# zyc-123/InstanceDiff

Measured on AMD Instinct MI355X. Metric: denoising steps/sec (256x256 bs16), higher is better.
Workload: dtype f32; 1 GPU; 256x256 1-ch synthetic, 1000-step reverse chain, batch 16 per GPU, 2 UNet fwd + reverse update per step; global_batch=16, parallelism=replicas x1 (no collective)

## Files before the change

instancediff_amd/csrc/conv_wino4.hip:

```cpp
#include "conv_args.h"
#include "wino_common.h"

using idiff_detail::ConvArgs;

namespace {

using namespace idiff_wino;

constexpr int CK = 4;
constexpr int TW = 32, TH = 16;
constexpr int RCOLS = TW + 2;
constexpr int RS = 40;
constexpr int TRH = TH + 2;
constexpr int PS = TRH * RS;
constexpr int PSP = 768;
constexpr int NT = 512;
constexpr int NL = 6;
constexpr int R_FLOATS = NL * NT;
constexpr int V_FLOATS = 9 * 2 * 64 * 4;
constexpr int U_FLOATS = 9 * 4 * 64 * 4;

typedef float floatx2 __attribute__((ext_vector_type(2)));

template <bool UPSAMPLED>
constexpr unsigned long long chunk_live() {
    unsigned long long m = 0;
    for (int q = 0; q < 9; ++q) m |= (unsigned long long)quad_live<UPSAMPLED>(q) << (4 * q);
    return m;
}
template <bool UPSAMPLED>
constexpr unsigned chunk_sets() {
    unsigned m = 0, n = 0;
    for (int q = 0; q < 9; ++q) m |= (n & 1u) << q, n += quad_live<UPSAMPLED>(q) != 0;
    return m | (n & 1u) << 9;
}

struct Geo4 {
    int np;
    int total;
    int tiles_y8;
};

#ifdef IDIFF_WINO_SLOTS
#define SLOT_INIT long long sl_acc[10] = {0, 0, 0, 0, 0, 0, 0, 0, 0, 0}, sl_t = 0;
#define SLOT_START sl_t = __builtin_readcyclecounter();
#define SLOT_MARK(k)                                        \
    {                                                       \
        const long long t_ = __builtin_readcyclecounter();  \
        sl_acc[k] += t_ - sl_t;                             \
        sl_t = t_;                                          \
    }
#define SLOT_FINI                                                                                                                   \
    if (lane == 0) {                                                                                                                \
        long long w_ = 0;                                                                                                           \
        for (int q_ = 0; q_ < 9; ++q_) w_ += sl_acc[q_];                                                                            \
        atomicAdd((unsigned long long*)trace + 8 + 2 * wave, (unsigned long long)w_);                                               \
        atomicAdd((unsigned long long*)trace + 9 + 2 * wave, (unsigned long long)sl_acc[9]);                                        \
    }
#else
#define SLOT_INIT
#define SLOT_START
#define SLOT_MARK(k)
#define SLOT_FINI
#endif

template <int MODE, int SPEC, bool RAG, bool HEAVY, bool G16>
__device__ __forceinline__ void conv_wino4_body(const ConvArgs& a, const Geo4& g, float* smem TRACE_PARAM) {
    static_assert(!G16 || (MODE == IDIFF_CONV_NORMAL && SPEC != 2), "the 16-byte gather: contiguous pieces, LDS-DMA only");
    constexpr int HU = G16 ? 5 : 4, HR = 3;
    constexpr int N_U = HEAVY ? HU : 9 - HU;
    constexpr int NR = G16 ? (HEAVY ? HR : 3 - HR) : NL;
    constexpr bool UPS = MODE == IDIFF_CONV_UPSAMPLE2;
    float* const Rb = smem;
    float* const Vb = smem + 3 * R_FLOATS;
    float* const Ub = Vb + 2 * V_FLOATS;
    float* const econst = Ub + 2 * U_FLOATS;
    int* const gtab = reinterpret_cast<int*>(econst + 512);
    constexpr unsigned R_BYTES = R_FLOATS * 4, U_BYTES = U_FLOATS * 4;
    const unsigned lds_base = __builtin_amdgcn_readfirstlane((unsigned)reinterpret_cast<unsigned long long>(smem));
    const unsigned U_LDS0 = lds_base + (3 * R_FLOATS + 2 * V_FLOATS) * 4;

    const int tid = threadIdx.x;
    const int lane = tid & 63;
    const int wave = __builtin_amdgcn_readfirstlane(tid >> 6);
    const int k4 = lane >> 4;
    const int cb = wave & 3;
    const int tblk = wave >> 2;
    const int g16_u0 = HEAVY ? wave : 4 * HU + wave - 4, g16_r0 = HEAVY ? wave : 4 * HR + wave - 4;
    const int HWin = a.Hin * a.Win;
    const int nchunks = a.Cin / CK;

    constexpr int RSRC_FLAGS = 0x00020000;
    struct View {
        int b, co0, y0, x0;
    };
    const float *p0A = a.src0, *p1A = a.src0, *puA = a.wwino4, *p0B = a.src0, *p1B = a.src0, *puB = a.wwino4;
    View vA = {0, 0, 0, 0}, vB = {0, 0, 0, 0};
    int nrB = 0;
    unsigned omaskA = 0, omaskB = 0;
    int it_b = 0, it_cob = 0, it_px = 0, it_py = 0;
    const int tiles_y = g.np / a.tiles_x;
    int d_cob, d_px, d_py, d_b;
    {
        const int G0 = gridDim.x;
        d_cob = G0 % a.ncob;
        const int r1 = G0 / a.ncob;
        d_px = r1 % a.tiles_x;
        const int r2 = r1 / a.tiles_x;
        d_py = r2 % tiles_y;
        d_b = r2 / tiles_y;
    }
    auto decode_first = [&](int item) {
        it_cob = item % a.ncob;
        const int r1 = item / a.ncob;
        it_px = r1 % a.tiles_x;
        const int r2 = r1 / a.tiles_x;
        it_py = r2 % tiles_y;
        it_b = r2 / tiles_y;
    };
    auto advance_item = [&]() {
        it_cob += d_cob;
        int carry = it_cob >= a.ncob;
        it_cob -= carry ? a.ncob : 0;
        it_px += d_px + carry;
        carry = it_px >= a.tiles_x;
        it_px -= carry ? a.tiles_x : 0;
        it_py += d_py + carry;
        carry = it_py >= tiles_y;
        it_py -= carry ? tiles_y : 0;
        it_b += d_b + carry;
    };
    auto decode_B = [&]() {
        vB.b = it_b, vB.co0 = it_cob * 64, vB.y0 = it_py * TH, vB.x0 = it_px * TW;
        puB = scalar_ptr(a.wwino4 + (long long)it_cob * U_FLOATS);
        p0B = scalar_ptr(a.src0 + (long long)it_b * a.bs0);
        p1B = scalar_ptr(SPEC == 3 ? a.src1 + (long long)it_b * a.bs1 : a.src0);
        nrB = 0x7fffffff;
    };
    auto write_table = [&](const View& v) {
        unsigned om;
        if (G16) gather_decode16<NT, NR, 256, PSP / 4, PS / 4, RS / 4>(tid, g16_r0 * 64 + lane, om, v.y0, v.x0, a, gtab, HWin);
        else gather_decode<MODE, NT, NL, PSP, PS, RS, RCOLS>(tid, om, v.y0, v.x0, a, gtab, HWin);
        return om;
    };
    auto shift_B_to_A = [&]() { p0A = p0B, p1A = p1B, puA = puB, vA = vB, omaskA = omaskB; };
    const int ustride_b = a.ncob * U_FLOATS * 4;

    typedef const __attribute__((address_space(4))) floatx4* cfloatx4p;
    struct Pro {
        floatx4 a, b;
    };
    auto load_pro = [&](int p) {
        Pro r;
        if (SPEC == 2) {
            const bool inA = p < nchunks;
            const long long o = (long long)(inA ? vA.b : vB.b) * a.C0r + (inA ? p : p - nchunks) * CK;
            r.a = *(cfloatx4p)(a.pro_a + o);
            r.b = *(cfloatx4p)(a.pro_b + o);
        }
        return r;
    };

    const unsigned u_voff = tid * 16;
    const unsigned l_voff = lane * 16;
    auto dma_u_piece16 = [&](int p, int buf, int i) {
        const bool inA = p < nchunks;
        const unsigned ub = (unsigned)(g16_u0 + 4 * i) * 1024u;
        const int so = (inA ? p : p - nchunks) * ustride_b + (int)ub;
        const __amdgpu_buffer_rsrc_t rsu = __builtin_amdgcn_make_buffer_rsrc(const_cast<float*>(inA ? puA : puB), 0, inA ? 0x7fffffff : nrB, RSRC_FLAGS);
        const unsigned lds0 = __builtin_amdgcn_readfirstlane(U_LDS0 + (unsigned)buf * U_BYTES + ub);
        asm volatile("s_nop 4\n\ts_mov_b32 m0, %2\n\ts_nop 0\n\tbuffer_load_dwordx4 %0, %1, %3 offen lds" ::"v"(l_voff), "s"(rsu), "s"(lds0), "s"(so) : "memory");
    };
    auto dma_u = [&](int p, int buf) {
        if (G16) {
#pragma unroll
            for (int i = 0; i < N_U; ++i) dma_u_piece16(p, buf, i);
            return;
        }
        const bool inA = p < nchunks;
        const int so = (inA ? p : p - nchunks) * ustride_b;
        const __amdgpu_buffer_rsrc_t rsu = __builtin_amdgcn_make_buffer_rsrc(const_cast<float*>(inA ? puA : puB), 0, inA ? 0x7fffffff : nrB, RSRC_FLAGS);
        const unsigned lds0 = __builtin_amdgcn_readfirstlane(U_LDS0 + (unsigned)buf * U_BYTES + (unsigned)wave * 1024u);
        asm volatile(
            "s_nop 4\n\ts_mov_b32 m0, %2\n\ts_nop 0\n\tbuffer_load_dwordx4 %0, %1, %3 offen lds\n\t"
            "s_add_u32 m0, m0, 0x2000\n\ts_nop 0\n\tbuffer_load_dwordx4 %0, %1, %4 offen lds\n\t"
            "s_add_u32 m0, m0, 0x2000\n\ts_nop 0\n\tbuffer_load_dwordx4 %0, %1, %5 offen lds\n\t"
            "s_add_u32 m0, m0, 0x2000\n\ts_nop 0\n\tbuffer_load_dwordx4 %0, %1, %6 offen lds"
            ::"v"(u_voff), "s"(rsu), "s"(lds0), "s"(so), "s"(so + NT * 16), "s"(so + 2 * NT * 16), "s"(so + 3 * NT * 16)
            : "memory", "scc");
        if (!HEAVY) {
            const unsigned lds4 = __builtin_amdgcn_readfirstlane(lds0 + 4 * NT * 16 - 256 * 16);
            asm volatile("s_nop 4\n\ts_mov_b32 m0, %2\n\ts_nop 0\n\tbuffer_load_dwordx4 %0, %1, %3 offen lds" ::"v"(u_voff), "s"(rsu), "s"(lds4),
                         "s"(so + 4 * NT * 16 - 256 * 16)
                         : "memory");
        }
    };
    auto dma_u_piece = [&](int p, int buf, int i) {
        if (G16) return dma_u_piece16(p, buf, i);
        const bool inA = p < nchunks;
        const int so = (inA ? p : p - nchunks) * ustride_b + (i < 4 ? i * NT * 16 : 4 * NT * 16 - 256 * 16);
        const __amdgpu_buffer_rsrc_t rsu = __builtin_amdgcn_make_buffer_rsrc(const_cast<float*>(inA ? puA : puB), 0, inA ? 0x7fffffff : nrB, RSRC_FLAGS);
        const unsigned lds0 = __builtin_amdgcn_readfirstlane(U_LDS0 + (unsigned)buf * U_BYTES + (unsigned)wave * 1024u + (unsigned)(i < 4 ? i * NT * 16 : 4 * NT * 16 - 256 * 16));
        asm volatile("s_nop 4\n\ts_mov_b32 m0, %2\n\ts_nop 0\n\tbuffer_load_dwordx4 %0, %1, %3 offen lds" ::"v"(u_voff), "s"(rsu), "s"(lds0), "s"(so) : "memory");
    };
    auto dma_raw = [&](int p, unsigned rslot) {
        const bool inA = p < nchunks;
        const int cbase = (inA ? p : p - nchunks) * CK;
        int goff[NL];
#pragma unroll
        for (int i = 0; i < NL; ++i) goff[i] = gtab[i * NT + tid];
        const int C0v = a.C0v;
        const bool second = SPEC == 3 && cbase >= C0v;
        const unsigned long long b0 = reinterpret_cast<unsigned long long>(inA ? p0A : p0B), b1 = reinterpret_cast<unsigned long long>(inA ? p1A : p1B);
        const float* const base = reinterpret_cast<const float*>(second ? b1 : b0);
        const int so = (second ? cbase - C0v : cbase) * HWin * 4;
        const __amdgpu_buffer_rsrc_t rs = __builtin_amdgcn_make_buffer_rsrc(const_cast<float*>(base), 0, inA ? 0x7fffffff : nrB, RSRC_FLAGS);
        const unsigned lds0 = __builtin_amdgcn_readfirstlane(lds_base + rslot + (unsigned)wave * 256u);
        asm volatile(
            "s_nop 4\n\ts_mov_b32 m0, %8\n\ts_nop 0\n\tbuffer_load_dword %0, %6, %7 offen lds\n\t"
            "s_add_u32 m0, m0, 0x800\n\ts_nop 0\n\tbuffer_load_dword %1, %6, %7 offen lds\n\t"
            "s_add_u32 m0, m0, 0x800\n\ts_nop 0\n\tbuffer_load_dword %2, %6, %7 offen lds\n\t"
            "s_add_u32 m0, m0, 0x800\n\ts_nop 0\n\tbuffer_load_dword %3, %6, %7 offen lds\n\t"
            "s_add_u32 m0, m0, 0x800\n\ts_nop 0\n\tbuffer_load_dword %4, %6, %7 offen lds\n\t"
            "s_add_u32 m0, m0, 0x800\n\ts_nop 0\n\tbuffer_load_dword %5, %6, %7 offen lds"
            ::"v"(goff[0]), "v"(goff[1]), "v"(goff[2]), "v"(goff[3]), "v"(goff[4]), "v"(goff[5]), "s"(rs), "s"(so), "s"(lds0)
            : "memory", "scc");
    };
    auto dma_raw_piece = [&](int p, unsigned rslot, int i, int goff_i) {
        const bool inA = p < nchunks;
        const int cbase = (inA ? p : p - nchunks) * CK;
        const int C0v = a.C0v;
        const bool second = SPEC == 3 && cbase >= C0v;
        const unsigned long long b0 = reinterpret_cast<unsigned long long>(inA ? p0A : p0B), b1 = reinterpret_cast<unsigned long long>(inA ? p1A : p1B);
        const float* const base = reinterpret_cast<const float*>(second ? b1 : b0);
        const int so = (second ? cbase - C0v : cbase) * HWin * 4;
        const __amdgpu_buffer_rsrc_t rs = __builtin_amdgcn_make_buffer_rsrc(const_cast<float*>(base), 0, inA ? 0x7fffffff : nrB, RSRC_FLAGS);
        if (G16) {
            const unsigned lds16 = __builtin_amdgcn_readfirstlane(lds_base + rslot + (unsigned)(g16_r0 + 4 * i) * 1024u);
            asm volatile("s_nop 4\n\ts_mov_b32 m0, %3\n\ts_nop 0\n\tbuffer_load_dwordx4 %0, %1, %2 offen lds" ::"v"(goff_i), "s"(rs), "s"(so), "s"(lds16) : "memory");
            return;
        }
        const unsigned lds0 = __builtin_amdgcn_readfirstlane(lds_base + rslot + (unsigned)wave * 256u + (unsigned)i * 2048u);
        asm volatile("s_nop 4\n\ts_mov_b32 m0, %3\n\ts_nop 0\n\tbuffer_load_dword %0, %1, %2 offen lds" ::"v"(goff_i), "s"(rs), "s"(so), "s"(lds0) : "memory");
    };
    auto dma_raw_fill = [&](int p, unsigned rslot) {
        if (G16) {
#pragma unroll
            for (int i = 0; i < NR; ++i) dma_raw_piece(p, rslot, i, gtab[i * NT + tid]);
        } else {
            dma_raw(p, rslot);
        }
    };
    float rinA[NL], rinB[NL];
    auto ld_raw = [&](float (&dst)[NL], int p, int i, int goff_i) {
        const bool inA = p < nchunks;
        const int so = (inA ? p : p - nchunks) * CK * HWin * 4;
        const __amdgpu_buffer_rsrc_t rs = __builtin_amdgcn_make_buffer_rsrc(const_cast<float*>(inA ? p0A : p0B), 0, inA ? 0x7fffffff : nrB, RSRC_FLAGS);
        asm volatile("s_nop 4\n\tbuffer_load_dword %0, %1, %2, %3 offen" : "=v"(dst[i]) : "v"(goff_i), "s"(rs), "s"(so) : "memory");
    };
    auto stage_act = [&](const float (&src)[NL], int p, const Pro& pro, unsigned rslot, int i0, int i1) {
        const unsigned om = p < nchunks ? omaskA : omaskB;
        float* const R = reinterpret_cast<float*>(reinterpret_cast<char*>(Rb) + rslot) + tid;
        constexpr bool hiw = !HEAVY;
#pragma unroll
        for (int i = 0; i < NL; ++i) {
            if (i < i0 || i >= i1) continue;
            const float pa = i == 0 ? pro.a.x : i == 1 ? (hiw ? pro.a.y : pro.a.x) : i == 2 ? pro.a.y : i == 3 ? pro.a.z : i == 4 ? (hiw ? pro.a.w : pro.a.z) : pro.a.w;
            const float pb = i == 0 ? pro.b.x : i == 1 ? (hiw ? pro.b.y : pro.b.x) : i == 2 ? pro.b.y : i == 3 ? pro.b.z : i == 4 ? (hiw ? pro.b.w : pro.b.z) : pro.b.w;
            const float x = silu_fast(pa * src[i] + pb);
            R[i * NT] = ((om >> i) & 1u) ? 0.f : x;
        }
    };

    constexpr bool heavy = HEAVY;
    const int trole = wave & 1;
    const int thalf = (wave >> 1) & 1;
    const int tx = lane & 7, tyl = (lane >> 3) & 1;
    const float al = trole ? -1.f : -4.f, be = trole ? 2.f : 1.f;
    const float* const trbase = Rb + k4 * PSP + (4 * (2 * thalf + tyl) + (heavy ? 1 : trole)) * RS + 4 * tx;
    const int ufirst = heavy ? 1 + 2 * trole : 5 * trole;
    float* const vwbase = Vb + thalf * 256 + lane * 4;
    float ta[6], tb[6], tlo[6], thi[6];
    struct Row16 {
        floatx4 lo, mid, hi;
    };
    Row16 ra, rb;
    auto rd_row = [&](const float* p, float (&d)[6], Row16& w) {
        if (G16) {
            w.lo = *reinterpret_cast<const floatx4*>(p);
            w.mid = *reinterpret_cast<const floatx4*>(p + 4);
            w.hi = *reinterpret_cast<const floatx4*>(p + 8);
            return;
        }
        const floatx4 lo = *reinterpret_cast<const floatx4*>(p);
        const floatx2 hi = *reinterpret_cast<const floatx2*>(p + 4);
        d[0] = lo.x, d[1] = lo.y, d[2] = lo.z, d[3] = lo.w, d[4] = hi.x, d[5] = hi.y;
    };
    auto take_row = [&](float (&d)[6], Row16& w) {
        if (!G16) return;
        asm volatile("" : "+v"(w.lo), "+v"(w.hi));
        d[0] = w.lo.w, d[1] = w.mid.x, d[2] = w.mid.y, d[3] = w.mid.z, d[4] = w.mid.w, d[5] = w.hi.x;
    };
    auto tr_piece = [&](int piece, unsigned rslot, int buf) {
        const float* p = reinterpret_cast<const float*>(reinterpret_cast<const char*>(trbase) + rslot);
        if (piece == 0) {
            if (heavy) rd_row(p + 1 * RS, ta, ra), rd_row(p + 3 * RS, tb, rb);
            else rd_row(p, ta, ra), rd_row(p + 2 * RS, tb, rb);
        } else if (piece == 1) {
            take_row(ta, ra), take_row(tb, rb);
            if (heavy) {
#pragma unroll
                for (int c = 0; c < 6; ++c) tlo[c] = __builtin_fmaf(al, ta[c], tb[c]);
                rd_row(p, ta, ra), rd_row(p + 2 * RS, tb, rb);
            } else {
#pragma unroll
                for (int c = 0; c < 6; ++c) tlo[c] = __builtin_fmaf(4.f, ta[c], -5.f * tb[c]);
                rd_row(p + 4 * RS, ta, ra);
            }
        } else if (piece == 2) {
            take_row(ta, ra);
            if (heavy) take_row(tb, rb);
            if (heavy) {
                if (UPS && !trole) {
#pragma unroll
                    for (int c = 0; c < 6; ++c) tlo[c] = __builtin_fmaf(be, __builtin_fmaf(al, ta[c], tb[c]), tlo[c]);
                } else {
#pragma unroll
                    for (int c = 0; c < 6; ++c) {
                        const float X = tlo[c], Y = __builtin_fmaf(al, ta[c], tb[c]);
                        tlo[c] = __builtin_fmaf(be, Y, X);
                        thi[c] = __builtin_fmaf(-be, Y, X);
                    }
                }
            } else {
#pragma unroll
                for (int c = 0; c < 6; ++c) tlo[c] += ta[c];
            }
        } else {
            const int which = piece - 3;
            if (which == 1 && !heavy) return;
            if (UPS && which == 1 && !trole) return;
            float o[6];
            bt6<UPS>(which ? thi : tlo, o);
            const int u = ufirst + which;
            float* const V = vwbase + buf * V_FLOATS;
            *reinterpret_cast<floatx4*>(V + PF(u) * 512) = floatx4{o[0], o[1], o[2], o[3]};
            *reinterpret_cast<floatx2*>(V + PH(u) * 512 + 2 * (u & 1)) = floatx2{o[4], o[5]};
        }
    };

    const int G = gridDim.x;
    const int first = (int)xcd_remap(blockIdx.x, G);
    const int last = g.total;
    if (first >= last) return;
    auto fetch_consts = [&](const View& v) {
        float e = 0.f;
        if (HEAVY) {
            const int which = tid >> 6, co = v.co0 + (tid & 63);
            if (co < a.Cout) {
                if (which == 0 && a.bias) e = a.bias[co];
                if (which == 1 && a.vec) e = a.vec[(long long)v.b * a.Cout + co];
                if (which == 2 && a.aux) e = a.aux_a[(long long)v.b * a.Cout + co];
                if (which == 3 && a.aux) e = a.aux_b[(long long)v.b * a.Cout + co];
            }
        }
        return e;
    };
    TRACE_INIT(8)
    SLOT_INIT

    decode_first(first);
    decode_B();
    shift_B_to_A();
    omaskA = write_table(vA);
    if (first + G < last) {
        advance_item();
        decode_B();
    } else {
        nrB = 0, vB = vA;
    }
    {
        const float e0 = fetch_consts(vA);
        if (HEAVY) econst[tid] = e0;
    }
    dma_u(0, 0);
    if (SPEC != 2) {
        dma_raw_fill(0, 0 * R_BYTES);
        dma_raw_fill(1, 1 * R_BYTES);
        dma_raw_fill(2, 2 * R_BYTES);
        asm volatile("s_waitcnt vmcnt(%0)" ::"n"(NR) : "memory");
        __syncthreads();
    } else {
        int goff[NL];
#pragma unroll
        for (int i = 0; i < NL; ++i) goff[i] = gtab[i * NT + tid];
#pragma unroll
        for (int i = 0; i < NL; ++i) ld_raw(rinA, 0, i, goff[i]);
#pragma unroll
        for (int i = 0; i < NL; ++i) ld_raw(rinB, 1, i, goff[i]);
        const Pro pro0 = load_pro(0), pro1 = load_pro(1);
        asm volatile("s_waitcnt vmcnt(0)" : "+v"(rinA[0]), "+v"(rinA[1]), "+v"(rinA[2]), "+v"(rinA[3]), "+v"(rinA[4]), "+v"(rinA[5]), "+v"(rinB[0]),
                     "+v"(rinB[1]), "+v"(rinB[2]), "+v"(rinB[3]), "+v"(rinB[4]), "+v"(rinB[5])::"memory");
        stage_act(rinA, 0, pro0, 0 * R_BYTES, 0, NL);
        stage_act(rinB, 1, pro1, 1 * R_BYTES, 0, NL);
#pragma unroll
        for (int i = 0; i < NL; ++i) ld_raw(rinA, 2, i, goff[i]);
        __syncthreads();
    }
#pragma unroll
    for (int piece = 0; piece < 5; ++piece) tr_piece(piece, 0 * R_BYTES, 0);
    if (SPEC == 2) asm volatile("s_waitcnt vmcnt(0)" : "+v"(rinA[0]), "+v"(rinA[1]), "+v"(rinA[2]), "+v"(rinA[3]), "+v"(rinA[4]), "+v"(rinA[5])::"memory");
    else asm volatile("s_waitcnt vmcnt(0)" ::: "memory");
    __syncthreads();
    dma_u(1, 1);

    unsigned r_t = 1 * R_BYTES, r_a = 2 * R_BYTES, r_x = 0 * R_BYTES;
    int epar = 0;
    bool young = false;
    for (int item = first; item < last; item += G) {
        TRACE_MARK(0)
        TRACE_LAP(3)
        floatx4 acc[36];
        {
            const int opoff = lane * 4;
            floatx4 ob[2], oa[2];
            ob[0] = *reinterpret_cast<const floatx4*>(Vb + tblk * 256 + opoff);
            oa[0] = *reinterpret_cast<const floatx4*>(Ub + cb * 256 + opoff);
            auto chunk = [&](int cc, auto par_tag, auto zero_tag) {
                constexpr int PAR = decltype(par_tag)::value;
                constexpr bool ZERO = decltype(zero_tag)::value;
                const float* V = Vb + PAR * V_FLOATS + tblk * 256 + opoff;
                const float* U = Ub + PAR * U_FLOATS + cb * 256 + opoff;
                constexpr unsigned long long LIVE = chunk_live<UPS>();
                constexpr unsigned SETS = chunk_sets<UPS>();
                static_assert((LIVE >> 32) != 0 && (LIVE & 0xf) != 0, "quads 0 and 8 carry the chunk's first and last operand requests");
                auto qlive = [](int q) { return (unsigned)(LIVE >> (4 * q)) & 0xfu; };
                auto qset = [](int q, int par) { return (int)(((SETS >> q) ^ ((SETS >> 9) & (unsigned)par)) & 1u); };
                const float* Vn = Vb + (PAR ^ 1) * V_FLOATS + tblk * 256 + opoff;
                const float* Un = Ub + (PAR ^ 1) * U_FLOATS + cb * 256 + opoff;
                int goff[NL];
                if (cc + 3 == nchunks) omaskB = write_table(vB);
#pragma unroll
                for (int i = 0; i < NL; ++i) goff[i] = i < NR ? gtab[i * NT + tid] : 0;
                float(&rin_s)[NL] = PAR ? rinB : rinA;
                float(&rin_l)[NL] = PAR ? rinA : rinB;
                Pro pro;
                if (SPEC == 2) pro = load_pro(cc + 2);
                SLOT_START
#pragma unroll
                for (int q = 0; q < 9; ++q) {
                    const unsigned lm = qlive(q);
                    if (q + 1 < 9) {
                        if (lm) {
                            const int nq = qlive(q + 1) ? q + 1 : q + 2;
                            ob[qset(nq, PAR)] = *reinterpret_cast<const floatx4*>(V + nq * 512);
                            oa[qset(nq, PAR)] = *reinterpret_cast<const floatx4*>(U + nq * 1024);
                        }
                    } else {
                        if (young) asm volatile("s_waitcnt vmcnt(%0)" ::"n"(NR + (RAG ? 0 : 16)) : "memory");
                        else asm volatile("s_waitcnt vmcnt(%0)" ::"n"(NR) : "memory");
                        young = false;
                        __builtin_amdgcn_sched_barrier(0);
                        SLOT_MARK(8)
                        __syncthreads();
                        SLOT_MARK(9)
                        if (cc + 1 == nchunks) dma_u(cc + 2, PAR);
                        else dma_u_piece(cc + 2, PAR, 0);
                        ob[qset(0, PAR ^ 1)] = *reinterpret_cast<const floatx4*>(Vn);
                        oa[qset(0, PAR ^ 1)] = *reinterpret_cast<const floatx4*>(Un);
                    }
                    if (lm) {
                        const floatx4 bv = ob[qset(q, PAR)], av = oa[qset(q, PAR)];
                        const floatx4 z4 = floatx4{0.f, 0.f, 0.f, 0.f};
                        if (lm & 1u) acc[4 * q + 0] = __builtin_amdgcn_mfma_f32_16x16x4f32(av.x, bv.x, ZERO ? z4 : acc[4 * q + 0], 0, 0, 0);
                        if (lm & 2u) acc[4 * q + 1] = __builtin_amdgcn_mfma_f32_16x16x4f32(av.y, bv.y, ZERO ? z4 : acc[4 * q + 1], 0, 0, 0);
                        if (lm & 4u) acc[4 * q + 2] = __builtin_amdgcn_mfma_f32_16x16x4f32(av.z, bv.z, ZERO ? z4 : acc[4 * q + 2], 0, 0, 0);
                        if (lm & 8u) acc[4 * q + 3] = __builtin_amdgcn_mfma_f32_16x16x4f32(av.w, bv.w, ZERO ? z4 : acc[4 * q + 3], 0, 0, 0);
                    }
                    if (!ZERO) {
                        if (!G16) {
                            if (q < 3) dma_u_piece(cc + 1, PAR ^ 1, q + 1);
                            if (q == 3 && !HEAVY) dma_u_piece(cc + 1, PAR ^ 1, 4);
                        }
                    }
                    if (SPEC == 2 && q == 5) {
                        if (young) asm volatile("s_waitcnt vmcnt(%6)" : "+v"(rin_s[0]), "+v"(rin_s[1]), "+v"(rin_s[2]), "+v"(rin_s[3]), "+v"(rin_s[4]), "+v"(rin_s[5]) : "n"(N_U + 2 + (RAG ? 0 : 16)) : "memory");
                        else asm volatile("s_waitcnt vmcnt(%6)" : "+v"(rin_s[0]), "+v"(rin_s[1]), "+v"(rin_s[2]), "+v"(rin_s[3]), "+v"(rin_s[4]), "+v"(rin_s[5]) : "n"(N_U + 2) : "memory");
                        stage_act(rin_s, cc + 2, pro, r_a, 0, 2);
                    }
                    if (SPEC == 2 && q == 6) stage_act(rin_s, cc + 2, pro, r_a, 2, 4);
                    if (SPEC == 2 && q == 7) stage_act(rin_s, cc + 2, pro, r_a, 4, 6);
                    auto req = [&](int i) {
                        if (SPEC == 2) ld_raw(rin_l, cc + 3, i, goff[i]);
                        else dma_raw_piece(cc + 3, r_x, i, goff[i]);
                    };
                    if (G16) {
                        static_assert(!G16 || N_U - 1 + NR <= 8, "a piece at quad 8 would lie behind the counted wait");
                        if (q < N_U - 1) {
                            if (!ZERO) dma_u_piece(cc + 1, PAR ^ 1, q + 1);
                        } else if (q < N_U - 1 + NR) {
                            req(q - (N_U - 1));
                        }
                    } else {
                        if (HEAVY && q == 3) req(0);
                        if (!HEAVY && q == 4) req(0);
                        if (q == 4) req(1);
                        if (q == 5) req(2);
                        if (q == 6) req(3);
                        if (q == 7) req(4), req(5);
                    }
                    if (q < 5) tr_piece(q, r_t, PAR ^ 1);
                    __builtin_amdgcn_sched_barrier(0);
                    if (q < 8) { SLOT_MARK(q) }
                }
                const unsigned t = r_t;
                r_t = r_a, r_a = r_x, r_x = t;
            };
            chunk(0, std::integral_constant<int, 0>{}, std::true_type{});
            chunk(1, std::integral_constant<int, 1>{}, std::false_type{});
            for (int cc = 2; cc < nchunks; cc += 2) {
                chunk(cc, std::integral_constant<int, 0>{}, std::false_type{});
                chunk(cc + 1, std::integral_constant<int, 1>{}, std::false_type{});
            }
        }
        TRACE_MARK(1)

        const View v = vA;
        const float* const ebase_item = econst + epar * 256;
        const bool more = item + G < last;
        float pre_e = 0.f;
        if (more) {
            shift_B_to_A();
            if (item + 2 * G < last) {
                advance_item();
                decode_B();
            } else {
                nrB = 0, vB = vA;
            }
            pre_e = fetch_consts(vA);
        }
        young = true;

        const int b = v.b, co0 = v.co0, y0 = v.y0, x0 = v.x0;
        {
            int lane_e = lane;
            asm volatile("" : "+v"(lane_e));
            const int j = lane_e & 15, k4 = lane_e >> 4;
            const int HWo = a.Hout * a.Wout;
            const int ty0 = y0 + 8 * tblk;
            const bool wave_live = co0 + cb * 16 < a.Cout;
            const long long wave_org = (long long)(co0 + cb * 16) * HWo + (long long)ty0 * a.Wout + x0;
            const __amdgpu_buffer_rsrc_t rso = __builtin_amdgcn_make_buffer_rsrc(const_cast<float*>(scalar_ptr(a.out + (long long)b * a.obs + wave_org)), 0, wave_live ? 0x7fffffff : 0, RSRC_FLAGS);
            const float* const resb = a.res ? a.res + (long long)b * a.rbs + wave_org : nullptr;
            const float* const auxb = a.aux ? a.aux + (long long)b * a.abs_ + wave_org : nullptr;
            const bool inside = !RAG || ((ty0 + 4 * (j >> 3) < a.Hout) && (x0 + 4 * (j & 7) < a.Wout));
            const unsigned lane_off = (unsigned)(4 * k4) * (unsigned)HWo + (unsigned)(4 * (j >> 3)) * (unsigned)a.Wout + 4u * (j & 7);
            const float* const ebase = ebase_item + cb * 16 + 4 * k4;
            const bool want_stats = a.stats != nullptr && ty0 < a.Hout && wave_live;
            const bool has_res = a.res != nullptr && wave_live, has_aux = a.aux != nullptr && wave_live;
            const float* const stbase = a.stats ? a.stats + (((long long)b * a.ntiles + (ty0 >> 3) * a.tiles_x + (x0 >> 5)) * a.Cout + co0 + cb * 16) * 2 : a.out;
            const __amdgpu_buffer_rsrc_t rst = __builtin_amdgcn_make_buffer_rsrc(const_cast<float*>(scalar_ptr(stbase)), 0, want_stats ? 0x7fffffff : 0, RSRC_FLAGS);
            constexpr int AUX_SC1 = 1 << 4;
            float zz[6][4][4];
            auto m = [&](int u, int v, int r) { return pos_live<UPS>(u, v) ? acc[pos(u, v)][r] : 0.f; };
#pragma unroll
            for (int u = 0; u < 6; ++u) {
                if (UPS && u == 2) continue;
#pragma unroll
                for (int r = 0; r < 4; ++r) {
                    at6(m(u, 0, r), m(u, 1, r), m(u, 2, r), m(u, 3, r), m(u, 4, r), m(u, 5, r), zz[u][r]);
                    asm volatile("" : "+v"(zz[u][r][0]), "+v"(zz[u][r][1]), "+v"(zz[u][r][2]), "+v"(zz[u][r][3]));
                }
                __builtin_amdgcn_sched_barrier(0);
            }
            TRACE_MARK(2)
            floatx4 nres = floatx4{0.f, 0.f, 0.f, 0.f}, naux = nres;
#ifdef W4_STATS_LAST
            typedef unsigned uintx2_ __attribute__((ext_vector_type(2)));
            uintx2_ spr[4];
#endif
            auto fetch = [&](int s) {
                if (!inside) return;
                const long long so = (long long)(s >> 2) * HWo + (s & 3) * a.Wout;
                if (has_res) nres = *reinterpret_cast<const floatx4*>(resb + so + lane_off);
                if (has_aux) naux = *reinterpret_cast<const floatx4*>(auxb + so + lane_off);
            };
            fetch(0);
#pragma unroll
            for (int r = 0; r < 4; ++r) {
                const float bv = ebase[r];
                float y[4][4];
#pragma unroll
                for (int x = 0; x < 4; ++x) {
                    float col[4];
                    at6(zz[0][r][x], zz[1][r][x], UPS ? 0.f : zz[2][r][x], zz[3][r][x], zz[4][r][x], zz[5][r][x], col);
#pragma unroll
                    for (int dy = 0; dy < 4; ++dy) y[dy][x] = col[dy] + bv;
                }
                {
                    float ssum = 0.f, ssq = 0.f;
                    if (a.stats != nullptr) {
#pragma unroll
                        for (int dy = 0; dy < 4; ++dy) {
                            ssum += (y[dy][0] + y[dy][1]) + (y[dy][2] + y[dy][3]);
                            ssq += (y[dy][0] * y[dy][0] + y[dy][1] * y[dy][1]) + (y[dy][2] * y[dy][2] + y[dy][3] * y[dy][3]);
                        }
                        if (!inside) ssum = 0.f, ssq = 0.f;
                        ssum = row_sum16(ssum);
                        ssq = row_sum16(ssq);
                    }
                    typedef unsigned uintx2 __attribute__((ext_vector_type(2)));
                    const uintx2 pr = {__builtin_bit_cast(unsigned, ssum), __builtin_bit_cast(unsigned, ssq)};
#ifndef W4_STATS_LAST
                    __builtin_amdgcn_raw_buffer_store_b64(pr, rst, j == 15 ? (4 * k4 + r) * 8 : -1, 0, AUX_SC1);
#else
                    spr[r] = pr;
#endif
                }
                const float add = ebase[64 + r];
                float aa = 0.f, ab = 0.f;
                if (has_aux) aa = ebase[128 + r], ab = ebase[192 + r];
#pragma unroll
                for (int dy = 0; dy < 4; ++dy) {
                    const floatx4 cres = nres, caux = naux;
                    if (4 * r + dy + 1 < 16) fetch(4 * r + dy + 1);
                    floatx4 v4 = floatx4{y[dy][0] + add, y[dy][1] + add, y[dy][2] + add, y[dy][3] + add};
                    if (has_res) v4 += cres;
                    if (has_aux) {
                        v4.x += silu_fast(aa * caux.x + ab), v4.y += silu_fast(aa * caux.y + ab);
                        v4.z += silu_fast(aa * caux.z + ab), v4.w += silu_fast(aa * caux.w + ab);
                    }
                    typedef unsigned uintx4 __attribute__((ext_vector_type(4)));
                    if (!RAG || inside) __builtin_amdgcn_raw_buffer_store_b128(__builtin_bit_cast(uintx4, v4), rso, (int)(lane_off * 4u), (r * HWo + dy * a.Wout) * 4, 0);
                }
                __builtin_amdgcn_sched_barrier(0);
            }
#ifdef W4_STATS_LAST
#pragma unroll
            for (int r = 0; r < 4; ++r) __builtin_amdgcn_raw_buffer_store_b64(spr[r], rst, j == 15 ? (4 * k4 + r) * 8 : -1, 0, AUX_SC1);
#endif
        }
        TRACE_MARK(3)
        if (HEAVY && more) econst[(epar ^ 1) * 256 + tid] = pre_e;
        epar ^= 1;
    }
    asm volatile("s_waitcnt vmcnt(0)" ::: "memory");
    TRACE_FINI(8)
    SLOT_FINI
}

template <int MODE, int SPEC, bool RAG>
__global__ __launch_bounds__(NT) void conv_wino4_kernel(const ConvArgs a, const Geo4 g TRACE_PARAM) {
    extern __shared__ __attribute__((aligned(16))) float smem[];
#ifdef IDIFF_WINO_TRACE
    if (__builtin_amdgcn_readfirstlane(threadIdx.x >> 6) < 4) conv_wino4_body<MODE, SPEC, RAG, true, false>(a, g, smem, trace);
    else conv_wino4_body<MODE, SPEC, RAG, false, false>(a, g, smem, trace);
#else
    if (__builtin_amdgcn_readfirstlane(threadIdx.x >> 6) < 4) conv_wino4_body<MODE, SPEC, RAG, true, false>(a, g, smem);
    else conv_wino4_body<MODE, SPEC, RAG, false, false>(a, g, smem);
#endif
}

template <int SPEC, bool RAG>
__global__ __launch_bounds__(NT) void conv_wino4_g16_kernel(const ConvArgs a, const Geo4 g TRACE_PARAM) {
    extern __shared__ __attribute__((aligned(16))) float smem[];
#ifdef IDIFF_WINO_TRACE
    if (__builtin_amdgcn_readfirstlane(threadIdx.x >> 6) < 4) conv_wino4_body<IDIFF_CONV_NORMAL, SPEC, RAG, true, true>(a, g, smem, trace);
    else conv_wino4_body<IDIFF_CONV_NORMAL, SPEC, RAG, false, true>(a, g, smem, trace);
#else
    if (__builtin_amdgcn_readfirstlane(threadIdx.x >> 6) < 4) conv_wino4_body<IDIFF_CONV_NORMAL, SPEC, RAG, true, true>(a, g, smem);
    else conv_wino4_body<IDIFF_CONV_NORMAL, SPEC, RAG, false, true>(a, g, smem);
#endif
}

template <auto KERN>
int launch_items(const ConvArgs& a, hipStream_t st) {
    const size_t lds = ((size_t)3 * R_FLOATS + 2 * V_FLOATS + 2 * U_FLOATS + 2 * 256 + NL * NT) * sizeof(float);
    static idiff_dyn_lds_cache lds_cache;
    auto kern = KERN;
    if (const int rc = idiff_dyn_lds(lds_cache, kern, lds, "conv2d(winograd4)")) return rc;
    int num_cu = 0;
    if (!idiff_num_cu(&num_cu)) IDIFF_FAIL(IDIFF_E_HIP, "conv2d(winograd4): cannot query the CU count");
    Geo4 g;
    const int tiles_y16 = (a.Hout + TH - 1) / TH;
    g.np = a.tiles_x * tiles_y16;
    g.tiles_y8 = (a.Hout + 7) / 8;
    const long long total = (long long)a.B * g.np * a.ncob;
    if (total >= (1ll << 31)) IDIFF_FAIL(IDIFF_E_BADARG, "conv2d(winograd4): grid too large");
    g.total = (int)total;
    int per = 0;
    const int grid = persistent_grid(g.total, num_cu, &per);
#ifdef IDIFF_WINO_TRACE
    static long long* tr = nullptr;
    if (!tr) (void)hipMalloc(&tr, 32 * sizeof(long long));
    (void)hipMemsetAsync(tr, 0, 32 * sizeof(long long), st);
    hipLaunchKernelGGL(kern, dim3(grid), dim3(NT), lds, st, a, g, tr);
    long long h[32];
    (void)hipMemcpyAsync(h, tr, sizeof(h), hipMemcpyDeviceToHost, st);
    (void)hipStreamSynchronize(st);
    fprintf(stderr, "[wino4 trace] Cin=%d Cout=%d H=%d items=%d per=%d | main loop %lld | switch + output transform %lld | statistics + stores %lld | to next item %lld (cycles/item, wave 0)\n",
            a.Cin, a.Cout, a.Hout, g.total, per, h[0] / g.total, h[1] / g.total, h[2] / g.total, h[3] / g.total);
#ifdef IDIFF_WINO_SLOTS
    {
        const long long nch = (long long)g.total * (a.Cin / CK - 1);
        fprintf(stderr, "[wino4 slots] Cin=%d H=%d work/barrier-wait cycles per chunk, waves 0..7:", a.Cin, a.Hout);
        for (int w = 0; w < 8; ++w) fprintf(stderr, " %lld/%lld", h[8 + 2 * w] / nch, h[9 + 2 * w] / nch);
        fprintf(stderr, "\n");
    }
#endif
#else
    hipLaunchKernelGGL(kern, dim3(grid), dim3(NT), lds, st, a, g);
#endif
    IDIFF_CHECK_LAUNCH("conv2d_fwd(winograd4)");
    return IDIFF_OK;
}

template <int MODE, int SPEC, bool RAG>
int launch_rag(const ConvArgs& a, hipStream_t st) {
    if constexpr (MODE == IDIFF_CONV_NORMAL && SPEC != 2) {
        const bool al0 = !(reinterpret_cast<uintptr_t>(a.src0) & 15) && !(a.bs0 & 3) && !(a.Win & 3);
        const bool al1 = SPEC != 3 || (!(reinterpret_cast<uintptr_t>(a.src1) & 15) && !(a.bs1 & 3));
        if (al0 && al1) return launch_items<conv_wino4_g16_kernel<SPEC, RAG>>(a, st);
    }
    return launch_items<conv_wino4_kernel<MODE, SPEC, RAG>>(a, st);
}

__global__ void pack_wino4_kernel(const float* __restrict__ w, float* __restrict__ out, int Cout, int Cin, int transpose) {
    const int Co = transpose ? Cin : Cout, Ci = transpose ? Cout : Cin;
    const int ncob = (Co + 63) / 64;
    const long long n = (long long)Co * Ci;
    for (long long i = blockIdx.x * (long long)blockDim.x + threadIdx.x; i < n; i += (long long)gridDim.x * blockDim.x) {
        const int co = i % Co, ci = i / Co;
        float gk[3][3];
        load_taps(w, Cin, co, ci, transpose, gk);
        float t[6][3];
#pragma unroll
        for (int q = 0; q < 3; ++q) {
            float o[6];
            g6(gk[0][q], gk[1][q], gk[2][q], o);
#pragma unroll
            for (int u = 0; u < 6; ++u) t[u][q] = o[u];
        }
        const int cc = ci >> 2, kk = ci & 3;
        const int cbk = co >> 6, col = co & 63, cb = col >> 4, i16 = col & 15;
        float* dst = out + ((long long)cc * ncob + cbk) * U_FLOATS + cb * 256 + (kk * 16 + i16) * 4;
#pragma unroll
        for (int u = 0; u < 6; ++u) {
            float o[6];
            g6(t[u][0], t[u][1], t[u][2], o);
#pragma unroll
            for (int v = 0; v < 6; ++v) {
                const int p = pos(u, v);
                dst[(p >> 2) * 1024 + (p & 3)] = o[v];
            }
        }
    }
}

int wino4_mode() {
    static const int m = [] {
        const char* e = getenv("IDIFF_WINOGRAD4");
        return e ? atoi(e) : 1;
    }();
    return m;
}
}

namespace idiff_detail {

long long conv_wino4_items(const ConvArgs& a, int ks, int mode, bool requested) {
    if (ks != 3 || !a.wwino4 || (wino4_mode() == 0 && !requested)) return 0;
    if (mode != IDIFF_CONV_NORMAL && mode != IDIFF_CONV_UPSAMPLE2) return 0;
    if (a.Cout % 16 || a.Cin % 8 || a.C0v % CK || (a.Hout & 3) || (a.Wout & 3) || a.Wout < 24) return 0;
    if ((long long)a.Cin * a.Hin * a.Win * 4 >= (1ll << 31)) return 0;
    if (144ll * a.Cin * a.ncob * 64 + U_FLOATS * 4 >= (1ll << 31)) return 0;
    if (mode == IDIFF_CONV_UPSAMPLE2 && (a.pro_a || a.src1)) return 0;
    if (a.pro_a && a.src1) return 0;
    if (a.pro_a && ((a.C0r & 3) || (reinterpret_cast<uintptr_t>(a.pro_a) & 15) || (reinterpret_cast<uintptr_t>(a.pro_b) & 15))) return 0;
    if ((reinterpret_cast<uintptr_t>(a.wwino4) & 15) != 0) return 0;
    if ((a.obs & 3) || (a.res && (a.rbs & 3)) || (a.aux && (a.abs_ & 3))) return 0;
    if ((reinterpret_cast<uintptr_t>(a.out) & 15) || (reinterpret_cast<uintptr_t>(a.res) & 15) || (reinterpret_cast<uintptr_t>(a.aux) & 15)) return 0;
    return (long long)a.tiles_x * ((a.Hout + TH - 1) / TH) * a.ncob;
}

int launch_conv_wino4(const ConvArgs& a, int mode, hipStream_t st) {
#ifdef W4_ONLY
    return launch_rag<IDIFF_CONV_NORMAL, 1, false>(a, st);
#else
    return launch_spec_ladder(mode, a.pro_a != nullptr, a.src1 != nullptr, a.Hout % TH || a.Wout % TW, [&](auto mode_tag, auto spec_tag, auto rag_tag) {
        return launch_rag<decltype(mode_tag)::value, decltype(spec_tag)::value, decltype(rag_tag)::value>(a, st);
    });
#endif
}

}

extern "C" int idiff_pack_conv_weight_wino4(const float* w, float* wwino4, int Cout, int Cin, int transpose, idiff_stream_t stream) {
    return pack_entry<36>("pack_conv_weight_wino4", pack_wino4_kernel, w, wwino4, Cout, Cin, transpose, stream);
}
```

instancediff_amd/csrc/wino_common.h:

```cpp
#pragma once
#include <stdlib.h>

#include <type_traits>

#include "common.h"

namespace idiff_detail {
bool winograd_disabled();
}

namespace idiff_wino {


template <int CTRL>
__device__ __forceinline__ float dpp_row_shr(float v) {
    return __builtin_bit_cast(float, __builtin_amdgcn_update_dpp(0, __builtin_bit_cast(int, v), CTRL, 0xf, 0xf, true));
}
__device__ __forceinline__ float row_sum16(float v) {
    v += dpp_row_shr<0x111>(v);
    v += dpp_row_shr<0x112>(v);
    v += dpp_row_shr<0x114>(v);
    v += dpp_row_shr<0x118>(v);
    return v;
}

template <typename T>
__device__ __forceinline__ T* scalar_ptr(const T* p) {
    const unsigned long long v = reinterpret_cast<unsigned long long>(p);
    const unsigned lo = __builtin_amdgcn_readfirstlane((unsigned)v), hi = __builtin_amdgcn_readfirstlane((unsigned)(v >> 32));
    return reinterpret_cast<T*>(((unsigned long long)hi << 32) | lo);
}


__host__ __device__ constexpr int PF(int u) { return (3 * u + 1) / 2; }
__host__ __device__ constexpr int PH(int u) { return 1 + 3 * (u / 2); }
__host__ __device__ constexpr int pos(int u, int v) { return v < 4 ? 4 * PF(u) + v : 4 * PH(u) + 2 * (u & 1) + (v - 4); }

template <bool UPSAMPLED>
__host__ __device__ constexpr bool pos_live(int u, int v) {
    return !UPSAMPLED || (u != 2 && v != 2);
}
template <bool UPSAMPLED>
__host__ __device__ constexpr unsigned quad_live(int quad) {
    unsigned m = 0;
    for (int u = 0; u < 6; ++u)
        for (int v = 0; v < 6; ++v)
            if (pos_live<UPSAMPLED>(u, v) && pos(u, v) / 4 == quad) m |= 1u << (pos(u, v) & 3);
    return m;
}

template <bool UPSAMPLED = false>
__device__ __forceinline__ void bt6(const float (&x)[6], float (&o)[6]) {
    o[0] = __builtin_fmaf(4.f, x[0], __builtin_fmaf(-5.f, x[2], x[4]));
    const float p = __builtin_fmaf(-4.f, x[2], x[4]), q = __builtin_fmaf(-4.f, x[1], x[3]);
    o[1] = p + q;
    o[2] = UPSAMPLED ? p : p - q;
    const float c = x[4] - x[2], e = x[3] - x[1];
    o[3] = __builtin_fmaf(2.f, e, c);
    o[4] = __builtin_fmaf(-2.f, e, c);
    o[5] = __builtin_fmaf(4.f, x[1], __builtin_fmaf(-5.f, x[3], x[5]));
}
__device__ __forceinline__ void at6(const float x0, const float x1, const float x2, const float x3, const float x4, const float x5, float (&o)[4]) {
    const float s1 = x1 + x2, d1 = x1 - x2, s2 = x3 + x4, d2 = x3 - x4;
    o[0] = (x0 + s1) + s2;
    o[1] = __builtin_fmaf(2.f, d2, d1);
    o[2] = __builtin_fmaf(4.f, s2, s1);
    o[3] = __builtin_fmaf(8.f, d2, d1) + x5;
}
__device__ __forceinline__ void a6(float x0, float x1, float x2, float x3, float (&o)[6]) {
    const float s = x0 + x2, t = x1 + x3;
    o[0] = x0;
    o[1] = s + t;
    o[2] = s - t;
    const float p = __builtin_fmaf(4.f, x2, x0), q = __builtin_fmaf(8.f, x3, 2.f * x1);
    o[3] = p + q;
    o[4] = p - q;
    o[5] = x3;
}
__device__ __forceinline__ void g6(float x0, float x1, float x2, float (&o)[6]) {
    o[0] = 0.25f * x0;
    const float s = x0 + x2;
    o[1] = (-1.f / 6.f) * (s + x1);
    o[2] = (-1.f / 6.f) * (s - x1);
    const float t = __builtin_fmaf(4.f, x2, x0);
    o[3] = (1.f / 24.f) * __builtin_fmaf(2.f, x1, t);
    o[4] = (1.f / 24.f) * __builtin_fmaf(-2.f, x1, t);
    o[5] = x2;
}
__device__ __forceinline__ void gt3(float m0, float m1, float m2, float m3, float m4, float m5, float (&o)[3]) {
    const float s12 = m1 + m2, d12 = m1 - m2, s34 = m3 + m4, d34 = m3 - m4;
    o[0] = __builtin_fmaf(0.25f, m0, __builtin_fmaf(-1.f / 6.f, s12, (1.f / 24.f) * s34));
    o[1] = __builtin_fmaf(-1.f / 6.f, d12, (1.f / 12.f) * d34);
    o[2] = __builtin_fmaf(-1.f / 6.f, s12, __builtin_fmaf(1.f / 6.f, s34, m5));
}

template <int MODE, int NT, int NL, int PSP, int PS, int RS, int RCOLS, typename Args>
__device__ __forceinline__ void gather_decode(const int& tid, unsigned& om, const int& y0, const int& x0, const Args& a, int* const& gtab, const int& HWin) {
    int t = tid;
    asm volatile("" : "+v"(t));
    om = 0;
#pragma unroll
    for (int i = 0; i < NL; ++i) {
        const int e = t + i * NT;
        const int ci = e / PSP;
        const int rem = e - ci * PSP;
        const int r = rem / RS;
        const int c = rem - r * RS;
        const int oy = y0 - 1 + r, ox = x0 - 1 + c;
        const bool in = rem < PS && c < RCOLS && (unsigned)oy < (unsigned)a.Hout && (unsigned)ox < (unsigned)a.Wout;
        const int sp = MODE == IDIFF_CONV_UPSAMPLE2 ? (oy >> 1) * a.Win + (ox >> 1) : oy * a.Win + ox;
        gtab[i * NT + tid] = in ? (ci * HWin + sp) * 4 : -1;
        om |= (in ? 0u : 1u) << i;
    }
}

template <int NT, int NR, int ES, int PSP4, int PS4, int RS4, typename Args>
__device__ __forceinline__ void gather_decode16(const int& tid, const int& e0, unsigned& om, const int& y0, const int& x0, const Args& a, int* const& gtab, const int& HWin) {
    int t = e0;
    asm volatile("" : "+v"(t));
    om = 0;
#pragma unroll
    for (int i = 0; i < NR; ++i) {
        const int e = t + i * ES;
        const int ci = e / PSP4;
        const int rem = e - ci * PSP4;
        const int r = rem / RS4;
        const int j = rem - r * RS4;
        const int oy = y0 - 1 + r, ox4 = x0 - 4 + 4 * j;
        const bool in = rem < PS4 && (unsigned)oy < (unsigned)a.Hout && (unsigned)ox4 < (unsigned)a.Wout;
        gtab[i * NT + tid] = in ? (ci * HWin + oy * a.Win + ox4) * 4 : -1;
        om |= (in ? 0u : 1u) << i;
    }
}

__device__ __forceinline__ void load_taps(const float* __restrict__ w, int Cin, int co, int ci, int transpose, float (&g)[3][3]) {
#pragma unroll
    for (int p = 0; p < 3; ++p)
#pragma unroll
        for (int q = 0; q < 3; ++q)
            g[p][q] = transpose ? w[((long long)ci * Cin + co) * 9 + (2 - p) * 3 + (2 - q)] : w[((long long)co * Cin + ci) * 9 + p * 3 + q];
}


template <int NPOS, typename K>
int pack_entry(const char* name, K kern, const float* w, float* image, int Cout, int Cin, int transpose, idiff_stream_t stream) {
    IDIFF_CHECK_ARG(w && image && Cout > 0 && Cin > 0, "%s: bad args", name);
    const int Co = transpose ? Cin : Cout, Ci = transpose ? Cout : Cin;
    IDIFF_CHECK_ARG(Co % 16 == 0 && Ci % 8 == 0, "%s: needs conv Cout %% 16 == 0 and Cin %% 8 == 0 (got %d, %d)", name, Co, Ci);
    if (Co % 64) {
        hipError_t e = hipMemsetAsync(image, 0, (size_t)NPOS * Ci * ((Co + 63) / 64) * 64 * sizeof(float), (hipStream_t)stream);
        if (e != hipSuccess) IDIFF_FAIL(IDIFF_E_HIP, "%s: hipMemsetAsync: %s", name, hipGetErrorString(e));
    }
    const long long n = (long long)Cout * Cin;
    const int grid = (int)((n + 255) / 256 > 4096 ? 4096 : (n + 255) / 256);
    hipLaunchKernelGGL(kern, dim3(grid), dim3(256), 0, (hipStream_t)stream, w, image, Cout, Cin, transpose);
    IDIFF_CHECK_LAUNCH(name);
    return IDIFF_OK;
}

inline int persistent_grid(int total, int slots, int* per_out = nullptr) {
    const int per = (total + slots - 1) / slots;
    if (per_out) *per_out = per;
    return (total + per - 1) / per;
}

template <typename F>
int launch_spec_ladder(int mode, bool pro, bool src1, bool ragged, F&& launch) {
    auto rag = [&](auto mode_tag, auto spec_tag) {
        if (ragged) return launch(mode_tag, spec_tag, std::true_type{});
        return launch(mode_tag, spec_tag, std::false_type{});
    };
    using Normal = std::integral_constant<int, IDIFF_CONV_NORMAL>;
    using Upsample = std::integral_constant<int, IDIFF_CONV_UPSAMPLE2>;
    if (mode == IDIFF_CONV_UPSAMPLE2) return rag(Upsample{}, std::integral_constant<int, 1>{});
    if (pro) return rag(Normal{}, std::integral_constant<int, 2>{});
    if (src1) return rag(Normal{}, std::integral_constant<int, 3>{});
    return rag(Normal{}, std::integral_constant<int, 1>{});
}

}

#ifdef IDIFF_WINO_TRACE
#define TRACE_PARAM , long long* trace
#define TRACE_INIT(N) long long tr_t[(N) + 1] = {0}, tr_acc[N] = {0};
#define TRACE_MARK(k)                       \
    tr_t[k] = __builtin_readcyclecounter(); \
    if (k > 0) tr_acc[k - 1] += tr_t[k] - tr_t[k - 1];
#define TRACE_LAP(last) \
    if (tr_t[last] != 0) tr_acc[last] += tr_t[0] - tr_t[last];
#define TRACE_FINI(N)                                                                                                   \
    if (tid == 0) {                                                                                                     \
        for (int q_ = 0; q_ < (N); ++q_) atomicAdd((unsigned long long*)trace + q_, (unsigned long long)tr_acc[q_]);    \
    }
#else
#define TRACE_PARAM
#define TRACE_INIT(N)
#define TRACE_MARK(k)
#define TRACE_LAP(last)
#define TRACE_FINI(N)
#endif
```

Measured before the change: 44.96 steps/s.

## Enable 16-byte vector gather path for prologue (SPEC 2) Winograd convolutions

Extends the 16-byte aligned gather path to the SPEC==2 variant, which applies a fused scale/shift plus SiLU prologue to the input. Instead of six scalar dword loads per thread, it issues dwordx4 buffer loads into registers, applies the prologue on the vectors and writes them to LDS. The wait and stage points are rescheduled inside the chunk loop, and the heavy/light work split is made configurable through macros. Out-of-range entries use a 0x80000000 offset so the buffer loads return zero. This aims to cut the number of global load instructions and the waits on them for prologue convolutions, at the cost of more vector registers and more complex vmcnt accounting.

```diff
diff --git a/instancediff_amd/csrc/conv_wino4.hip b/instancediff_amd/csrc/conv_wino4.hip
--- a/instancediff_amd/csrc/conv_wino4.hip
+++ b/instancediff_amd/csrc/conv_wino4.hip
@@ -19,6 +19,12 @@
 constexpr int R_FLOATS = NL * NT;
 constexpr int V_FLOATS = 9 * 2 * 64 * 4;
 constexpr int U_FLOATS = 9 * 4 * 64 * 4;
+#ifndef W4_P16_HU
+#define W4_P16_HU 5
+#endif
+#ifndef W4_P16_HR
+#define W4_P16_HR 2
+#endif
 
 typedef float floatx2 __attribute__((ext_vector_type(2)));
 
@@ -66,8 +72,9 @@
 
 template <int MODE, int SPEC, bool RAG, bool HEAVY, bool G16>
 __device__ __forceinline__ void conv_wino4_body(const ConvArgs& a, const Geo4& g, float* smem TRACE_PARAM) {
-    static_assert(!G16 || (MODE == IDIFF_CONV_NORMAL && SPEC != 2), "the 16-byte gather: contiguous pieces, LDS-DMA only");
-    constexpr int HU = G16 ? 5 : 4, HR = 3;
+    static_assert(!G16 || MODE == IDIFF_CONV_NORMAL, "the 16-byte gather: contiguous pieces");
+    constexpr int HU = G16 ? (SPEC == 2 ? W4_P16_HU : 5) : 4, HR = SPEC == 2 ? W4_P16_HR : 3;
+    static_assert(HU >= 4 && HU <= 5 && HR >= 1 && HR <= 3, "the dealings that build");
     constexpr int N_U = HEAVY ? HU : 9 - HU;
     constexpr int NR = G16 ? (HEAVY ? HR : 3 - HR) : NL;
     constexpr bool UPS = MODE == IDIFF_CONV_UPSAMPLE2;
@@ -139,7 +146,8 @@
     };
     auto write_table = [&](const View& v) {
         unsigned om;
-        if (G16) gather_decode16<NT, NR, 256, PSP / 4, PS / 4, RS / 4>(tid, g16_r0 * 64 + lane, om, v.y0, v.x0, a, gtab, HWin);
+        if (G16 && SPEC == 2) gather_decode16<NT, NR, 256, PSP / 4, PS / 4, RS / 4, (int)0x80000000>(tid, g16_r0 * 64 + lane, om, v.y0, v.x0, a, gtab, HWin);
+        else if (G16) gather_decode16<NT, NR, 256, PSP / 4, PS / 4, RS / 4>(tid, g16_r0 * 64 + lane, om, v.y0, v.x0, a, gtab, HWin);
         else gather_decode<MODE, NT, NL, PSP, PS, RS, RCOLS>(tid, om, v.y0, v.x0, a, gtab, HWin);
         return om;
     };
@@ -271,6 +279,30 @@
             R[i * NT] = ((om >> i) & 1u) ? 0.f : x;
         }
     };
+    floatx4 qinA[3], qinB[3];
+    auto ld_raw16 = [&](floatx4 (&dst)[3], int p, int i, int goff_i) {
+        const bool inA = p < nchunks;
+        const int so = (inA ? p : p - nchunks) * CK * HWin * 4;
+        const __amdgpu_buffer_rsrc_t rs = __builtin_amdgcn_make_buffer_rsrc(const_cast<float*>(inA ? p0A : p0B), 0, inA ? 0x7fffffff : nrB, RSRC_FLAGS);
+        asm volatile("s_nop 4\n\tbuffer_load_dwordx4 %0, %1, %2, %3 offen" : "=v"(dst[i]) : "v"(goff_i), "s"(rs), "s"(so) : "memory");
+    };
+    auto stage_act16 = [&](const floatx4 (&src)[3], int p, const Pro& pro, unsigned rslot, int i) {
+        const unsigned om = p < nchunks ? omaskA : omaskB;
+        const int piece = g16_r0 + 4 * i, ch = piece / 3;
+        const float pa = ch == 0 ? pro.a.x : ch == 1 ? pro.a.y : ch == 2 ? pro.a.z : pro.a.w;
+        const float pb = ch == 0 ? pro.b.x : ch == 1 ? pro.b.y : ch == 2 ? pro.b.z : pro.b.w;
+        const floatx4 s = src[i];
+        floatx4 x = floatx4{silu_fast(pa * s.x + pb), silu_fast(pa * s.y + pb), silu_fast(pa * s.z + pb), silu_fast(pa * s.w + pb)};
+        if ((om >> i) & 1u) x = floatx4{0.f, 0.f, 0.f, 0.f};
+        *reinterpret_cast<floatx4*>(reinterpret_cast<char*>(Rb) + rslot + (unsigned)piece * 1024u + l_voff) = x;
+    };
+#define W4_WAIT16(q, n)                                                                                                    \
+    {                                                                                                                      \
+        if (NR == 1) asm volatile("s_waitcnt vmcnt(%1)" : "+v"(q[0]) : "n"(n) : "memory");                                 \
+        else if (NR == 2) asm volatile("s_waitcnt vmcnt(%2)" : "+v"(q[0]), "+v"(q[1]) : "n"(n) : "memory");                \
+        else if (NR == 3) asm volatile("s_waitcnt vmcnt(%3)" : "+v"(q[0]), "+v"(q[1]), "+v"(q[2]) : "n"(n) : "memory");    \
+        else asm volatile("s_waitcnt vmcnt(%0)" ::"n"(n) : "memory");                                                      \
+    }
 
     constexpr bool heavy = HEAVY;
     const int trole = wave & 1;
@@ -390,6 +422,23 @@
         dma_raw_fill(2, 2 * R_BYTES);
         asm volatile("s_waitcnt vmcnt(%0)" ::"n"(NR) : "memory");
         __syncthreads();
+    } else if (G16) {
+        int goff[3];
+#pragma unroll
+        for (int i = 0; i < NR; ++i) goff[i] = gtab[i * NT + tid];
+#pragma unroll
+        for (int i = 0; i < NR; ++i) ld_raw16(qinA, 0, i, goff[i]);
+#pragma unroll
+        for (int i = 0; i < NR; ++i) ld_raw16(qinB, 1, i, goff[i]);
+        const Pro pro0 = load_pro(0), pro1 = load_pro(1);
+        W4_WAIT16(qinA, 0) W4_WAIT16(qinB, 0)
+#pragma unroll
+        for (int i = 0; i < NR; ++i) stage_act16(qinA, 0, pro0, 0 * R_BYTES, i);
+#pragma unroll
+        for (int i = 0; i < NR; ++i) stage_act16(qinB, 1, pro1, 1 * R_BYTES, i);
+#pragma unroll
+        for (int i = 0; i < NR; ++i) ld_raw16(qinA, 2, i, goff[i]);
+        __syncthreads();
     } else {
         int goff[NL];
 #pragma unroll
@@ -409,7 +458,8 @@
     }
 #pragma unroll
     for (int piece = 0; piece < 5; ++piece) tr_piece(piece, 0 * R_BYTES, 0);
-    if (SPEC == 2) asm volatile("s_waitcnt vmcnt(0)" : "+v"(rinA[0]), "+v"(rinA[1]), "+v"(rinA[2]), "+v"(rinA[3]), "+v"(rinA[4]), "+v"(rinA[5])::"memory");
+    if (SPEC == 2 && G16) W4_WAIT16(qinA, 0)
+    else if (SPEC == 2) asm volatile("s_waitcnt vmcnt(0)" : "+v"(rinA[0]), "+v"(rinA[1]), "+v"(rinA[2]), "+v"(rinA[3]), "+v"(rinA[4]), "+v"(rinA[5])::"memory");
     else asm volatile("s_waitcnt vmcnt(0)" ::: "memory");
     __syncthreads();
     dma_u(1, 1);
@@ -444,6 +494,8 @@
                 for (int i = 0; i < NL; ++i) goff[i] = i < NR ? gtab[i * NT + tid] : 0;
                 float(&rin_s)[NL] = PAR ? rinB : rinA;
                 float(&rin_l)[NL] = PAR ? rinA : rinB;
+                floatx4(&qin_s)[3] = PAR ? qinB : qinA;
+                floatx4(&qin_l)[3] = PAR ? qinA : qinB;
                 Pro pro;
                 if (SPEC == 2) pro = load_pro(cc + 2);
                 SLOT_START
@@ -483,15 +535,26 @@
                             if (q == 3 && !HEAVY) dma_u_piece(cc + 1, PAR ^ 1, 4);
                         }
                     }
-                    if (SPEC == 2 && q == 5) {
+                    if (SPEC == 2 && !G16 && q == 5) {
                         if (young) asm volatile("s_waitcnt vmcnt(%6)" : "+v"(rin_s[0]), "+v"(rin_s[1]), "+v"(rin_s[2]), "+v"(rin_s[3]), "+v"(rin_s[4]), "+v"(rin_s[5]) : "n"(N_U + 2 + (RAG ? 0 : 16)) : "memory");
                         else asm volatile("s_waitcnt vmcnt(%6)" : "+v"(rin_s[0]), "+v"(rin_s[1]), "+v"(rin_s[2]), "+v"(rin_s[3]), "+v"(rin_s[4]), "+v"(rin_s[5]) : "n"(N_U + 2) : "memory");
                         stage_act(rin_s, cc + 2, pro, r_a, 0, 2);
                     }
-                    if (SPEC == 2 && q == 6) stage_act(rin_s, cc + 2, pro, r_a, 2, 4);
-                    if (SPEC == 2 && q == 7) stage_act(rin_s, cc + 2, pro, r_a, 4, 6);
+                    if (SPEC == 2 && !G16 && q == 6) stage_act(rin_s, cc + 2, pro, r_a, 2, 4);
+                    if (SPEC == 2 && !G16 && q == 7) stage_act(rin_s, cc + 2, pro, r_a, 4, 6);
+                    if (SPEC == 2 && G16 && NR > 0) {
+                        constexpr int QW = 8 - NR;
+                        constexpr int REQ_BEFORE = QW - (N_U - 1) < 0 ? 0 : QW - (N_U - 1) > NR ? NR : QW - (N_U - 1);
+                        static_assert(!(SPEC == 2 && G16) || N_U - 1 <= QW, "every copy of U(c+1) is issued before the wait");
+                        if (q == QW) {
+                            if (young) W4_WAIT16(qin_s, N_U + REQ_BEFORE + (RAG ? 0 : 16))
+                            else W4_WAIT16(qin_s, N_U + REQ_BEFORE)
+                        }
+                        if (q >= QW && q < 8) stage_act16(qin_s, cc + 2, pro, r_a, q - QW);
+                    }
                     auto req = [&](int i) {
-                        if (SPEC == 2) ld_raw(rin_l, cc + 3, i, goff[i]);
+                        if (SPEC == 2 && G16) ld_raw16(qin_l, cc + 3, i, goff[i]);
+                        else if (SPEC == 2) ld_raw(rin_l, cc + 3, i, goff[i]);
                         else dma_raw_piece(cc + 3, r_x, i, goff[i]);
                     };
                     if (G16) {
@@ -647,6 +710,7 @@
     asm volatile("s_waitcnt vmcnt(0)" ::: "memory");
     TRACE_FINI(8)
     SLOT_FINI
+#undef W4_WAIT16
 }
 
 template <int MODE, int SPEC, bool RAG>
@@ -717,7 +781,7 @@
 
 template <int MODE, int SPEC, bool RAG>
 int launch_rag(const ConvArgs& a, hipStream_t st) {
-    if constexpr (MODE == IDIFF_CONV_NORMAL && SPEC != 2) {
+    if constexpr (MODE == IDIFF_CONV_NORMAL) {
         const bool al0 = !(reinterpret_cast<uintptr_t>(a.src0) & 15) && !(a.bs0 & 3) && !(a.Win & 3);
         const bool al1 = SPEC != 3 || (!(reinterpret_cast<uintptr_t>(a.src1) & 15) && !(a.bs1 & 3));
         if (al0 && al1) return launch_items<conv_wino4_g16_kernel<SPEC, RAG>>(a, st);
diff --git a/instancediff_amd/csrc/wino_common.h b/instancediff_amd/csrc/wino_common.h
--- a/instancediff_amd/csrc/wino_common.h
+++ b/instancediff_amd/csrc/wino_common.h
@@ -114,7 +114,7 @@
     }
 }
 
-template <int NT, int NR, int ES, int PSP4, int PS4, int RS4, typename Args>
+template <int NT, int NR, int ES, int PSP4, int PS4, int RS4, int PAD = -1, typename Args>
 __device__ __forceinline__ void gather_decode16(const int& tid, const int& e0, unsigned& om, const int& y0, const int& x0, const Args& a, int* const& gtab, const int& HWin) {
     int t = e0;
     asm volatile("" : "+v"(t));
@@ -128,7 +128,7 @@
         const int j = rem - r * RS4;
         const int oy = y0 - 1 + r, ox4 = x0 - 4 + 4 * j;
         const bool in = rem < PS4 && (unsigned)oy < (unsigned)a.Hout && (unsigned)ox4 < (unsigned)a.Wout;
-        gtab[i * NT + tid] = in ? (ci * HWin + oy * a.Win + ox4) * 4 : -1;
+        gtab[i * NT + tid] = in ? (ci * HWin + oy * a.Win + ox4) * 4 : PAD;
         om |= (in ? 0u : 1u) << i;
     }
 }
```

Result: no change. 45.28 steps/s, median of 6 (+0.7%).
